# adolfogonzalez3/maddpg

Hardware: AMD Instinct MI355X
Metric: env-steps/sec (end-to-end at the reference update cadence), simple_spread N=3, batch 1024 (higher is better)
Workload: dtype fp32

## Files before the change

include/maddpg_hip.h:

```cpp
#ifndef MADDPG_HIP_H
#define MADDPG_HIP_H

#include <stddef.h>
#include <stdint.h>

#ifdef __cplusplus
extern "C" {
#endif

#define MDP_MAX_AGENTS 8
#define MDP_ACT_DIM 5
#define MDP_MAX_UNITS 256
#define MDP_ABI_VERSION 5

enum mdp_scenario {
    MDP_SCN_NONE = 0,
    MDP_SCN_SIMPLE = 1,
    MDP_SCN_SPREAD = 2,
    MDP_SCN_ADVERSARY = 3,
    MDP_SCN_TAG = 4,
    MDP_SCN_SPEAKER_LISTENER = 5
};

enum mdp_which {
// ... 162 lines not shown

int64_t mdp_td3_bytes(const mdp_config* cfg);
int mdp_td3_enable(mdp_handle* h, void* buf_dev, int64_t bytes, int32_t policy_delay);
int mdp_td3_info(mdp_handle* h, int32_t agent, double out4[4]);

int mdp_minimax_enable(mdp_handle* h, const float* eps_host);
int mdp_minimax_info(mdp_handle* h, float* eps_out_host);
int mdp_minimax_debug_adv(mdp_handle* h, float* critic_adv_dev, float* actor_adv_dev);

enum mdp_approx_set { MDP_APX_NET = 0, MDP_APX_TARGET = 1, MDP_APX_M = 2, MDP_APX_V = 3, MDP_APX_GRAD = 4 };
int64_t mdp_approx_bytes(const mdp_config* cfg);
int mdp_approx_enable(mdp_handle* h, void* buf_dev, int64_t bytes, float lambda);
int mdp_approx_set_params(mdp_handle* h, int32_t observer, int32_t agent, int32_t which, const float* src, int64_t n);
int mdp_approx_get_params(mdp_handle* h, int32_t observer, int32_t agent, int32_t which, float* dst, int64_t n);
int mdp_approx_get_beta_powers(mdp_handle* h, int32_t observer, int32_t agent, float out2[2]);
int mdp_approx_set_beta_powers(mdp_handle* h, int32_t observer, int32_t agent, const float in2[2]);
int mdp_approx_info(mdp_handle* h, int32_t observer, int32_t agent, double out4[4]);
int mdp_approx_logits(mdp_handle* h, int32_t observer, int32_t agent, int32_t target, const float* obs_dev,
                      float* logits_dev, int32_t rows);
int mdp_approx_grad(mdp_handle* h, int32_t observer, const int32_t* idx_dev);
int mdp_approx_step(mdp_handle* h, int32_t observer, const int32_t* idx_dev);

enum mdp_kernel_kind {
    MDP_K_INDEX = 0, MDP_K_GATHER = 1, MDP_K_CRITIC_GRAD = 2, MDP_K_ACTOR_GRAD = 3,
    MDP_K_APPLY = 4, MDP_K_ROLLOUT = 5, MDP_K_REDUCE = 6, MDP_K_REDUCE_APPLY = 7,
    MDP_K_ALLREDUCE = 8,
    MDP_K_PER_SYNC = 9, MDP_K_PER_SAMPLE = 10, MDP_K_PER_UPDATE = 11,
    MDP_K_EVAL = 12,
    MDP_K_COUNT = 13
};
int mdp_prof_enable(mdp_handle* h, int32_t kind, int32_t on);
int mdp_grad_variant(mdp_handle* h, int32_t agent);
int mdp_grad_twin(mdp_handle* h);
int mdp_prof_read(mdp_handle* h, int32_t kind, double* total_ms, int64_t* launches);

#ifdef __cplusplus
}
#endif
#endif
```

maddpg_amd/_lib.py:

```python
import ctypes
import os
import re

import torch

HERE = os.path.dirname(os.path.abspath(__file__))
LIB_PATH = os.environ.get("MDP_LIB") or os.path.join(HERE, "libmaddpg_hip.so")
HEADER = os.path.join(os.path.dirname(HERE), "include", "maddpg_hip.h")

MAX_AGENTS = 8
ACT_DISCRETE, ACT_BOX = 0, 1
ACT_DIM = 5
BENCH_W = 8
MAX_UNITS = 256
ABI_VERSION = 5

SCN = {"none": 0, "simple": 1, "simple_spread": 2, "simple_adversary": 3, "simple_tag": 4,
       "simple_speaker_listener": 5}
WHICH = {"actor": 0, "critic": 1, "tgt_actor": 2, "tgt_critic": 3, "m_actor": 4, "v_actor": 5,
         "m_critic": 6, "v_critic": 7, "g_actor": 8, "g_critic": 9,
         "critic2": 10, "tgt_critic2": 11, "m_critic2": 12, "v_critic2": 13, "g_critic2": 14}
APX_WHICH = {"net": 0, "tgt": 1, "m": 2, "v": 3, "grad": 4}
REGION = {"theta": 0, "target": 1, "adam_m": 2, "adam_v": 3, "grad": 4, "replay": 5, "index": 6,
          "stats": 7, "env": 8, "eplog": 9, "beta": 10, "slab": 11, "ctl": 12}
# ... 60 lines not shown
    "mdp_synchronize": (ctypes.c_int, [_P]),
    "mdp_region": (ctypes.c_int, [_P, _I32, ctypes.POINTER(_I64), ctypes.POINTER(_I64)]),
    "mdp_tensor": (ctypes.c_int, [_P, _I32, _I32, _I32, ctypes.POINTER(MdpTensorInfo)]),
    "mdp_row_layout": (ctypes.c_int, [_P, _I32, _I32P]),
    "mdp_set_act_dims": (ctypes.c_int, [_P, _I32P]),
    "mdp_get_act_dims": (ctypes.c_int, [_P, _I32P]),
    "mdp_set_act_spaces": (ctypes.c_int, [_P, _I32P, _I32P]),
    "mdp_get_act_spaces": (ctypes.c_int, [_P, _I32P, _I32P]),
    "mdp_set_params": (ctypes.c_int, [_P, _I32, _I32, _F32P, _I64]),
    "mdp_get_params": (ctypes.c_int, [_P, _I32, _I32, _F32P, _I64]),
    "mdp_get_beta_powers": (ctypes.c_int, [_P, _I32, _I32, _F32P]),
    "mdp_set_beta_powers": (ctypes.c_int, [_P, _I32, _I32, _F32P]),
    "mdp_buffer_len": (_I64, [_P]),
    "mdp_buffer_add_rows": (ctypes.c_int, [_P, _P, _I64]),
    "mdp_buffer_put_agent": (ctypes.c_int, [_P, _I32, _P, _P, _I64]),
    "mdp_buffer_set_len": (ctypes.c_int, [_P, _I64, _I64]),
    "mdp_buffer_set_ring": (ctypes.c_int, [_P, _I64, _I64, _I64]),
    "mdp_seed_py_random": (ctypes.c_int, [_P, ctypes.c_uint64]),
    "mdp_set_rng_state": (ctypes.c_int, [_P, _U32P]),
    "mdp_get_rng_state": (ctypes.c_int, [_P, _U32P]),
    "mdp_make_index": (ctypes.c_int, [_P, _I32, _P]),
    "mdp_sample_rows": (ctypes.c_int, [_P, _P, _I32, _P]),
    "mdp_act": (ctypes.c_int, [_P, _I32, _I32, _P, _P, _I32, _P]),
    "mdp_actor_logits": (ctypes.c_int, [_P, _I32, _I32, _P, _P, _I32]),
    "mdp_q_values": (ctypes.c_int, [_P, _I32, _I32, _P, _P, _I32]),
    "mdp_update": (ctypes.c_int, [_P, _I32, _P, _P, _P]),
    "mdp_update_gate": (ctypes.c_int, [_P, _I64]),
    "mdp_update_round": (ctypes.c_int, [_P]),
    "mdp_set_graphs": (ctypes.c_int, [_P, _I32]),
    "mdp_train_step": (ctypes.c_int, [_P, _I32]),
    "mdp_dp_unique_id": (ctypes.c_int, [ctypes.c_char_p]),
    "mdp_grad_variant": (ctypes.c_int, [_P, _I32]),
    "mdp_grad_twin": (ctypes.c_int, [_P]),
    "mdp_dp_init": (ctypes.c_int, [_P, ctypes.c_char_p, _I32, _I32]),
    "mdp_dp_xgmi_open": (ctypes.c_int, [_P, _I32, _I32, ctypes.c_char_p]),
    "mdp_dp_xgmi_connect": (ctypes.c_int, [_P, ctypes.c_char_p]),
    "mdp_dp_xgmi_probe": (ctypes.c_int, [_P, _I32P]),
    "mdp_dp_xgmi_enable": (ctypes.c_int, [_P]),
    "mdp_dp_xgmi_close": (ctypes.c_int, [_P]),
    "mdp_dp_info": (ctypes.c_int, [_P, _I32P]),
    "mdp_dp_exchange_stats": (ctypes.c_int, [_P, ctypes.POINTER(ctypes.c_double), _I32]),
    "mdp_dp_exchange_stats_enable": (ctypes.c_int, [_P, _I32]),
    "mdp_train_steps": (ctypes.c_int, [_P, _I32, ctypes.POINTER(ctypes.c_int32), _I32]),
    "mdp_agent_update": (ctypes.c_int, [_P, _I32, ctypes.c_int64, _P, _P, ctypes.POINTER(ctypes.c_double)]),
    "mdp_ra_plan": (ctypes.c_int, [ctypes.POINTER(MdpConfig), _I32, _I32, _I32P]),
    "mdp_critic_grad": (ctypes.c_int, [_P, _I32, _P, _P]),
    "mdp_actor_grad": (ctypes.c_int, [_P, _I32, _P, _P]),
    "mdp_reduce_grad": (ctypes.c_int, [_P, _I32, _I32]),
    "mdp_apply_grad": (ctypes.c_int, [_P, _I32, _I32, ctypes.c_float]),
    "mdp_get_stats": (ctypes.c_int, [_P, _I32, _F64P]),
    "mdp_check_finite": (ctypes.c_int, [_P, ctypes.POINTER(_I64)]),
    "mdp_env_reset": (ctypes.c_int, [_P]),
    "mdp_env_step": (ctypes.c_int, [_P, _P, _P]),
    "mdp_env_get_state": (ctypes.c_int, [_P, _F32P, _F32P, _I32P, _I32P]),
    "mdp_env_set_state": (ctypes.c_int, [_P, _F32P, _F32P, _I32P, _I32P]),
    "mdp_env_get_comm": (ctypes.c_int, [_P, _F32P]),
    "mdp_env_set_comm": (ctypes.c_int, [_P, _F32P]),
    "mdp_env_obs": (ctypes.c_int, [_P, _P]),
    "mdp_env_step_bench": (ctypes.c_int, [_P, _P]),
    "mdp_env_step_bench_u": (ctypes.c_int, [_P, _P, _P]),
    "mdp_evaluate": (ctypes.c_int, [_P, _I64, _I32, _I32, _P, _P, _P]),
    "mdp_evaluate_q": (ctypes.c_int, [_P, _I64, _I32, _I32, _I32, _I32, _P, _P, _P, _P, _P]),
    "mdp_eval_initial_state": (ctypes.c_int, [_P, _I64, _I32, _F32P, _F32P, _I32P]),
    "mdp_actor_set_floats": (_I64, [_P]),
    "mdp_actor_set_write": (ctypes.c_int, [_P, _P, _I32, _F32P, _I64]),
    "mdp_actor_set_snapshot": (ctypes.c_int, [_P, _P]),
# ... 79 lines not shown
```

maddpg_amd/csrc/mdp_api.cpp:

```cpp
#include <hip/hip_runtime.h>

#include <algorithm>
#include <cmath>
#include <cstdio>
#include <cstdlib>
#include <cstring>
#include <string>
#include <dlfcn.h>
#include <rccl/rccl.h>

#include <map>
#include <vector>

#include "mdp_kernels.h"
#include "mdp_variants.h"

namespace {

inline int64_t r4(int64_t n) { return (n + 3) & ~int64_t(3); }
inline int64_t a256(int64_t n) { return (n + 255) & ~int64_t(255); }

NDesc make_net(int64_t& off, int in, int H, int out) {
  NDesc d;
  d.off = (int)off;
// ... 251 lines not shown
}

struct mdp_handle {
  mdp_config cfg;
  Layout L;
  int device = 0;
  hipStream_t stream = nullptr;
  bool own_stream = false;
  char* arena = nullptr;
  float *theta, *target, *m, *v, *grad, *replay, *beta, *slab_c, *slab_a, *eplog;
  float *pos, *vel, *ep_rew;
  float* env_comm = nullptr;
  int32_t *index, *goal, *ep_step;
  double *stats, *stat_c, *stat_a, *y;
  Ctl* ctl;
  int64_t len = 0, next = 0;
  uint32_t act_ctr = 0, reset_ctr = 0;
  bool env_lockstep = true;
  std::string err;
  bool ready = false;
  bool prof_on[MDP_K_COUNT] = {};
  std::vector<hipEvent_t> ev[MDP_K_COUNT];
  size_t ev_used[MDP_K_COUNT] = {};
  double prof_ms[MDP_K_COUNT] = {};
  int64_t prof_n[MDP_K_COUNT] = {};
  bool graphs = true;
  bool capturing = false;
  int eager_rounds = 0;
  bool general_grads = false;
  bool box = false;
  bool fused_apply = true;
  bool ra_lanes = true;
  bool grad_twin = true;
  uint32_t* ra_ctr = nullptr;
  uint64_t* ra_part = nullptr;
  float* apre = nullptr;
  bool actor_pre = true;
  float* cpre = nullptr;
  bool critic_pre = true;
  float* apre_rows = nullptr;
  float* cpre_rows = nullptr;
  std::map<std::vector<int>, hipGraphExec_t> graph_exec;
  int eager_steps = 0;
  ncclComm_t comm = nullptr;
  int dp_world = 1;
  bool dp_graphs = false;
  int update_mode = 0;
  FusedApplyArgs* tp_list = nullptr;
  RaBatch tp_batch;
  RaBatch tp_reduce, tp_step;
  int ra_cap = 0, ra_batch_cap = 0;
  bool tp_fits[4] = {true, true, true, true};
  std::vector<FusedApplyArgs> tp_host[4];
  RaBatch tp_xchg;
  RaBatch tp_pair[3][MDP_MAX_AGENTS];
  bool tp_pair_fits[3][MDP_MAX_AGENTS] = {};
  FusedApplyArgs tp_pair_host[3][MDP_MAX_AGENTS][2];
  bool rollout_draw = true;
  bool draw_ahead = true;
  bool grad_pair = true;
  uint64_t* xbuf = nullptr;
  int x_world = 0, x_rank = 0;
  std::vector<void*> x_opened;
  XchgDesc* xd_dev = nullptr;
  uint32_t* x_probe = nullptr;
  uint32_t x_probe_ep = 0;
// ... 415 lines not shown
    if (lds > MDP_LDS_BUDGET) return fail(h, "minimax critic step does not fit in LDS");
    for (int j = 0; j < MDP_MAX_AGENTS; ++j) m.eps[j] = h->mm_eps[agent][j];
    m.adv_out = h->mm_adv_c;
    HIPCHK(h, mdp_launch_critic_grad_mm(m, h->L.topo.H, lds, h->stream));
    return 0;
  }
  if (lds_critic_bytes(h->L.topo, a.group) > MDP_LDS_BUDGET) return fail(h, "critic step does not fit in LDS");
  if (apx_agent(h, agent) && !tp) {
    CriticArgsApx x;
    static_cast<CriticArgs&>(x) = a;
    x.apx_target = apx_base(h, agent, MDP_APX_TARGET);
    HIPCHK(h, mdp_launch_critic_grad_apx(x, h->L.topo.H, lds_critic_bytes(h->L.topo, a.group), h->stream));
    return 0;
  }
  if (h->variant == Variant::Per && !tp)
    HIPCHK(h, mdp_launch_critic_grad_per(per_critic_args(h, a), h->L.topo.H, lds_critic_bytes(h->L.topo, a.group),
                                         h->stream));
  else
    HIPCHK(h, mdp_launch_critic_grad(a, h->L.topo.H, lds_critic_bytes(h->L.topo, a.group), h->stream));
  return 0;
}

ActorArgs actor_args(mdp_handle* h, int agent, const int32_t* idx, const float* u_act, bool tp, bool apre,
                     int pre_next, const int32_t* pre_idx, bool shared) {
  ActorArgs a;
  a.apre = apre ? h->apre : nullptr;
  a.apre_rows = h->apre_rows;
  a.cpre = nullptr;
  a.cpre_rows = h->cpre_rows;
  a.cpre_agent = pre_next;
  a.cpre_idx = pre_idx;
  a.target = h->target;
  a.multi = tp ? 2 : 0;
  a.slab_agent_stride = 0;
  a.topo = h->L.topo;
  a.agent = agent;
  a.B = h->cfg.batch_size;
  a.theta = h->theta;
  a.replay = h->replay;
  a.idx = idx;
  a.u_act = u_act;
  a.seed = h->cfg.seed;
  a.ctl = h->ctl;
  a.neg_inv_b = -1.0f / (float)a.B;
  a.reg_scale = (float)(2.0 * (double)h->cfg.actor_reg / ((double)a.B * MDP_ACT_DIM));
  a.slab = h->slab_a;
  a.slab_stride = h->L.slab_a;
  a.slab_stat = h->stat_a;
  if (tp) {
    if (!shared) a.slab += (int64_t)agent * h->L.nwg * h->L.slab_a;
    a.slab_stat += (int64_t)agent * h->L.nwg * 8;
  }
  return a;
}

int do_actor_grad(mdp_handle* h, int agent, const int32_t* idx, const float* u_act, bool tp = false,
                  bool apre = false, int pre_next = -1, const int32_t* pre_idx = nullptr, bool shared = false) {
  ActorArgs a = actor_args(h, agent, idx, u_act, tp, apre, pre_next, pre_idx, shared);
  ProfScope p(h, MDP_K_ACTOR_GRAD);
  if (!tp && !h->general_grads && grads_r_ok(h->L.topo, agent)) {
    int lds = lds_actor_r_bytes(h->L.topo);
    if (pre_next >= 0) {
      a.cpre = h->cpre;
      lds = std::max(lds, lds_critic_pre_bytes(h->L.topo));
    }
    HIPCHK(h, mdp_launch_actor_grad_r(a, lds, h->stream));
    return 0;
  }
  if (mm_agent(h, agent) && !tp) {
    ActorArgsMm m;
    static_cast<ActorArgs&>(m) = a;
    for (int j = 0; j < MDP_MAX_AGENTS; ++j) m.eps[j] = h->mm_eps[agent][j];
    m.adv_out = h->mm_adv_a;
    HIPCHK(h, mdp_launch_actor_grad_mm(m, h->L.topo.H, lds_actor_mm_bytes(h->L.topo), h->stream));
    return 0;
  }
  HIPCHK(h, mdp_launch_actor_grad(a, h->L.topo.H, lds_actor_bytes(h->L.topo), h->stream));
  return 0;
}

struct OptNet {
  NDesc net, other;
  float *theta, *target, *m, *v, *grad;
  const float* slab;
  int slab_stride;
  float* beta;
  const double* slab_stat;
  const double* y;
  double* stats_out;
  uint32_t* ticket;
  uint32_t* ctr;
  uint64_t* part;
  int slot;
  int net_id;
  int polyak, stats_mode, bump_ctr;
  bool own;
};

// ... 540 lines not shown
    a.slab_stat = h->stat_c;
    a.y_out = h->y;
    a.group = 0;
    a.twin = 1;
    a.multi = n;
    a.slab_agent_stride = nwg * h->L.slab_c;
    ProfScope p(h, MDP_K_CRITIC_GRAD);
    HIPCHK(h, mdp_launch_critic_grad_r(a, lds_c, h->stream));
  }
  {
    ActorArgs a;
    a.apre = nullptr;
    a.apre_rows = nullptr;
    a.cpre = nullptr;
    a.cpre_rows = nullptr;
    a.cpre_agent = -1;
    a.cpre_idx = nullptr;
    a.target = h->target;
    a.topo = h->L.topo;
    a.agent = 0;
    a.B = h->cfg.batch_size;
    a.theta = h->theta;
    a.replay = h->replay;
    a.idx = idx;
    a.u_act = u_act;
    a.seed = h->cfg.seed;
    a.ctl = h->ctl;
    a.neg_inv_b = -1.0f / (float)a.B;
    a.reg_scale = (float)(2.0 * (double)h->cfg.actor_reg / ((double)a.B * MDP_ACT_DIM));
    a.slab = h->slab_a;
    a.slab_stride = h->L.slab_a;
    a.slab_stat = h->stat_a;
    a.multi = n;
    a.slab_agent_stride = nwg * h->L.slab_a;
    ProfScope p(h, MDP_K_ACTOR_GRAD);
    HIPCHK(h, mdp_launch_actor_grad_r(a, lds_actor_r_bytes(h->L.topo), h->stream));
  }
  return 0;
}

int launch_tp_pair(mdp_handle* h, int pp, int i, int32_t* piece) {
  const int B = h->cfg.batch_size;
  const int kind = pp == 1 ? MDP_K_REDUCE : MDP_K_REDUCE_APPLY;
  if (h->tp_pair_fits[pp][i]) {
    RaBatch rb = h->tp_pair[pp][i];
    if (piece) {
      rb.pf_out = piece;
      rb.pf_count = B;
      rb.pf_ctl = h->ctl;
    }
    ProfScope p(h, kind);
    HIPCHK(h, mdp_launch_reduce_apply_batch(rb, h->stream));
    return 0;
  }
  for (int k = 0; k < 2; ++k) {
    FusedApplyArgs f = h->tp_pair_host[pp][i][k];
    if (piece) {
      f.pf_out = piece + (k ? (B + 1) / 2 : 0);
      f.pf_count = k ? B - (B + 1) / 2 : (B + 1) / 2;
      f.pf_ctl = h->ctl;
    }
    ProfScope p(h, kind);
    HIPCHK(h, mdp_launch_reduce_apply(f, h->stream, h->ra_lanes));
  }
  return 0;
}
// ... 321 lines not shown
  std::string err;
  if (!build_layout(cfg, L, err) || cus < 0 || per_cu < 0) return -1;
  int fallback = 0;
  for (int i = 0; i < cfg->n_agents; ++i)
    for (int net = 0; net < 2; ++net) {
      const int g = mdp_ra_grid_of(L.topo, i, net);
      const bool ok = mdp_ra_fits(L.topo, i, net, cus * per_cu);
      if (out) out[2 * i + net] = ok ? g : -g;
      fallback += ok ? 0 : 1;
    }
  return fallback;
}

int mdp_create(const mdp_config* cfg, void* arena_dev, int64_t arena_bytes, void* hip_stream, mdp_handle** out) {
  if (!out) return -1;
  *out = nullptr;
  mdp_handle* h = new mdp_handle();
  std::string err;
  if (!build_layout(cfg, h->L, err)) {
    h->err = err;
    *out = h;
    return -1;
  }
  h->cfg = *cfg;
  {
    const char* g = getenv("MDP_GENERAL_GRADS");
    h->general_grads = g && g[0] == '1';
    const char* u = getenv("MDP_UNFUSED_APPLY");
    h->fused_apply = !(u && u[0] == '1');
    const char* rl = getenv("MDP_RA_LANES");
    h->ra_lanes = !(rl && rl[0] == '0');
    const char* gt = getenv("MDP_GRAD_TWIN");
    h->grad_twin = !(gt && gt[0] == '0');
    const char* rd = getenv("MDP_ROLLOUT_DRAW");
    h->rollout_draw = !(rd && rd[0] == '0');
    const char* da = getenv("MDP_DRAW_AHEAD");
    h->draw_ahead = !(da && da[0] == '0');
    const char* gp = getenv("MDP_GRAD_PAIR");
    h->grad_pair = !(gp && gp[0] == '0');
    const char* ap = getenv("MDP_ACTOR_PRE");
    h->actor_pre = !(ap && ap[0] == '0');
    const char* cp = getenv("MDP_CRITIC_PRE");
    h->critic_pre = !(cp && cp[0] == '0');
  }
  if (!arena_dev || arena_bytes < h->L.total) {
    h->err = "arena missing or too small";
    *out = h;
    return -1;
  }
  *out = h;
  HIPCHK(h, hipGetDevice(&h->device));
  if (need_dev(h, arena_dev, h->L.total, "mdp_create", "arena_dev", false)) return -1;
  {
    int cus = 0, per = 0, per_b = 0;
    HIPCHK(h, hipDeviceGetAttribute(&cus, hipDeviceAttributeMultiprocessorCount, h->device));
    HIPCHK(h, mdp_ra_occupancy(&per));
    HIPCHK(h, mdp_ra_batch_occupancy(&per_b));
    h->ra_cap = cus * per;
    h->ra_batch_cap = cus * per_b;
    int scratch = 0;
    HIPCHK(h, mdp_spin_kernels_scratch(&scratch));
    if (scratch > 0) h->ra_cap = h->ra_batch_cap = 0;
    if (2 * h->L.nwg + h->L.nwg + 1 > cus) h->grad_twin = false;
  }
  if (hip_stream) {
    h->stream = (hipStream_t)hip_stream;
  } else {
    HIPCHK(h, hipStreamCreateWithFlags(&h->stream, hipStreamNonBlocking));
    h->own_stream = true;
  }
  h->arena = (char*)arena_dev;
  auto R = [&](int r) { return (void*)(h->arena + h->L.off[r]); };
  h->theta = (float*)R(MDP_R_THETA);
  h->target = (float*)R(MDP_R_TARGET);
  h->m = (float*)R(MDP_R_ADAM_M);
  h->v = (float*)R(MDP_R_ADAM_V);
  h->grad = (float*)R(MDP_R_GRAD);
  h->replay = (float*)R(MDP_R_REPLAY);
  h->index = (int32_t*)R(MDP_R_INDEX);
  h->stats = (double*)R(MDP_R_STATS);
  h->eplog = (float*)R(MDP_R_EPLOG);
  h->beta = (float*)R(MDP_R_BETA);
  h->ctl = (Ctl*)R(MDP_R_CTL);
  {
    const int E = cfg->num_envs, ne = h->L.n_ent, n = cfg->n_agents;
    char* p = (char*)R(MDP_R_ENV);
    h->pos = (float*)p;
    p += 4 * (int64_t)E * ne * 2;
    h->vel = (float*)p;
    p += 4 * (int64_t)E * ne * 2;
    h->goal = (int32_t*)p;
    p += 4 * (int64_t)E;
    h->ep_step = (int32_t*)p;
    p += 4 * (int64_t)E;
    h->ep_rew = (float*)p;
    p += 4 * (int64_t)E * n;
// ... 501 lines not shown
static bool any_prof(const mdp_handle* h) {
  for (int k = 0; k < MDP_K_COUNT; ++k)
    if (h->prof_on[k]) return true;
  return false;
}

int mdp_update_round(mdp_handle* h) {
  MDP_NEED(h);
  if (h->len <= 0) return fail(h, "update round on an empty replay buffer");
  h->trained = true;
  if (!h->graphs || any_prof(h) || h->eager_rounds < 1) {
    ++h->eager_rounds;
    td3_begin(h);
    const int rc = round_launches(h);
    if (!rc) commit_rounds(h, 1);
    return rc;
  }
  hipGraphExec_t x = nullptr;
  const int rc = captured_graph(h, graph_key(h, 0, {}), [&] { return round_launches(h); }, &x);
  if (rc) return rc;
  HIPCHK(h, hipGraphLaunch(x, h->stream));
  commit_rounds(h, 1);
  return 0;
}

int mdp_grad_variant(mdp_handle* h, int32_t agent) {
  if (unusable(h) || agent < 0 || agent >= h->cfg.n_agents) return -1;
  return (!h->general_grads && grads_r_ok(h->L.topo, agent)) ? 1 : 0;
}

int mdp_grad_twin(mdp_handle* h) {
  if (unusable(h)) return -1;
  return h->grad_twin ? 2 : 1;
}

int mdp_dp_unique_id(uint8_t* out128) {
  if (!out128 || !rccl().ok) return -1;
  ncclUniqueId id;
  if (rccl().get_id(&id) != ncclSuccess) return -1;
  std::memcpy(out128, &id, sizeof(id));
  return 0;
}

int mdp_dp_init(mdp_handle* h, const uint8_t* id128, int32_t world, int32_t rank) {
  if (unusable(h) || !id128) return -1;
  if (gate(h, Seam::DpInit)) return -1;
  if (h->p2p || h->xbuf) return fail(h, "mdp_dp_init: the xGMI exchange is already set up");
  if (!rccl().ok) return fail(h, "librccl.so.1 could not be loaded");
  if (world < 1 || rank < 0 || rank >= world) return fail(h, "mdp_dp_init: bad world/rank");
  if (h->comm) return fail(h, "mdp_dp_init: already initialised");
  ncclUniqueId id;
  std::memcpy(&id, id128, sizeof(id));
  HIPCHK(h, hipSetDevice(h->device));
  const ncclResult_t r = rccl().init_rank(&h->comm, world, id, rank);
  if (r != ncclSuccess) {
    h->comm = nullptr;
    h->err = std::string("ncclCommInitRank: ") + rccl().err(r);
    return -1;
  }
  h->dp_world = world;
  const char* g = getenv("MDP_DP_GRAPHS");
  h->dp_graphs = g && g[0] == '1';
  destroy_graphs(h, false);
  return 0;
}

// ... 1245 lines not shown
```

maddpg_amd/csrc/mdp_grads_r.hip:

```cpp
#include "mdp_device.h"
#include "mdp_kernels.h"
#include "mdp_mt.h"

#define MDP_RW MDP_R

#ifdef MDP_BUDGET
#ifndef MDP_BUDGET_AGENT
#define MDP_BUDGET_AGENT 1
#endif
#define MDP_BUD_N 72
#define MDP_BUD_WG 256
__device__ unsigned long long g_bud[2][MDP_BUD_WG][MDP_BUD_N];
__shared__ int s_bud;
__shared__ unsigned long long s_bud_t[MDP_BUD_N];
__shared__ unsigned s_bud_cnt;
#ifndef MDP_BUDGET_REP
#define MDP_BUDGET_REP 1
#endif
__device__ __forceinline__ unsigned long long bud_now() {
  const unsigned long long t = __builtin_amdgcn_s_memtime();
#if MDP_BUDGET_REP > 1
  const unsigned long long t2 = __builtin_amdgcn_s_memtime();
  asm volatile("" ::"s"(t2));
#endif
  return t;
}
__device__ __forceinline__ unsigned long long bud_real() { return __builtin_amdgcn_s_memrealtime(); }
#define BUD(i)                                           \
  do {                                                   \
    const unsigned long long t__ = bud_now();            \
    if ((threadIdx.x & 63) == 0) s_bud_t[i] = t__;       \
  } while (0)
// ... 801 lines not shown
    if (tt == 0 && half == 0) {
      s_l = sum16(s_l);
      s_y = sum16(s_y);
      s_r = sum16(s_r);
      s_q = sum16(s_q);
      if (lane == 0) {
        double* st = slab_stat + (int64_t)bx * 8;
        st[0] = s_l;
        st[1] = s_y;
        st[2] = s_r;
        st[3] = s_q;
      }
    }
  }
  const int vw = wave + 8 * half, vn = 8 * twin;
  CRIT_T(0);
  wgrad_vwaves(h1c, LH, RH, d2, LD, RH, slab + nd.t[2].off, vw, vn);
  CRIT_T(1);
  wgrad_vwaves(rowbuf + xo_c, ldr, ka_c, d1, LD, RH, slab + nd.t[0].off, vw, vn);
  CRIT_T(2);
  if (kb_c) wgrad_vwaves(rowbuf + ag.act_off, ldr, kb_c, d1, LD, RH, slab + nd.t[0].off + ka_c * RH, vw, vn);
  CRIT_T(3);
  if (wave == 4) MDP_STAMPW(9);
  if (vw == vn - 3) colsum64(d2, LD, slab + nd.t[3].off);
  if (vw == vn - 1) colsum64(d1, LD, slab + nd.t[1].off);
  CRIT_T(4);
  MDP_STAMP(10);
  MDP_WG_END(0);
}


template <bool NARROW>
__global__ __launch_bounds__(512) void k_actor_grad_r(ActorArgs a) {
  MDP_KARG_TOUCH("s"(a.agent), "s"(a.slab_stride), "s"(a.cpre_agent), "s"(a.topo.n), "s"(gridDim.x));
  if constexpr (NARROW) MDP_KARG_TOUCH("s"(a.topo.act_w4));
  extern __shared__ __attribute__((aligned(16))) float lds[];
  __shared__ int rows_ready;
  __shared__ int fwd_issued;
  BUD_BEGIN(1, a.agent, a.multi);
  MDP_WG_START(1);
  MDP_TL(a.ctl, 2, 0);
  int agent = a.agent, bx = blockIdx.x;
  if (a.cpre) {
    const int nwg = (a.B + MDP_RW - 1) / MDP_RW;
    if (bx >= nwg) {
      MDP_TL_ROLE(2, 1);
      critic_pre_tile<NARROW>(a, lds, &rows_ready, bx - nwg);
      MDP_WG_END(1);
      return;
    }
  }
  if (a.multi > 1) {
    const int nwg = (a.B + MDP_RW - 1) / MDP_RW;
    agent = bx / nwg;
    bx -= agent * nwg;
  }
  const int32_t* idx = a.multi > 1 ? a.idx + (int64_t)agent * a.B : a.idx;
  const float* u_act = (a.multi > 1 && a.u_act) ? a.u_act + (int64_t)agent * a.B * MDP_ACT_DIM : a.u_act;
  const Topo& T = a.topo;
  MDP_KARG_TOUCH(MDP_KARG_ADESC(T.ag[agent]));
  const ADesc& ag = T.ag[agent];
  const NDesc& na = ag.actor;
  const NDesc& nc = ag.critic;
  const bool lq = ag.local_q != 0;
  const int ldr = lds_ld(T.row_stride);
  const int ka_c = lq ? ag.obs_dim : ag.cin;
  const int xo_c = lq ? ag.obs_off : 0;
  LdsCarve cv(lds);
  MDP_CARVE_ACTOR_R(MDP_CARVE_DECL, ldr)

  const int wave = __builtin_amdgcn_readfirstlane(threadIdx.x >> 6);
  const int lane = threadIdx.x & 63, r = lane & 15, kq = lane >> 4;
  const int r0 = bx * MDP_R;
  const int nvalid = min(MDP_R, a.B - r0);
  const uint32_t ctr = ctr_load(a.ctl) + (a.multi > 1 ? (uint32_t)agent : 0u);
  const float* P = a.theta;
  constexpr int KC = 28, KSC = KC / 4;
  const int64_t ao = a.multi > 1 ? (int64_t)agent : 0;
  float* slab = a.slab + ao * a.slab_agent_stride + (int64_t)bx * a.slab_stride - na.off;
  double* slab_stat = a.slab_stat + ao * (int64_t)((a.B + MDP_R - 1) / MDP_R) * 8;
  MDP_STAMP(16);
  if (threadIdx.x == 0) rows_ready = 0;
  if (threadIdx.x == 1) fwd_issued = 0;
  __syncthreads();

  double s_q = 0.0, s_p = 0.0;
// ... 38 lines not shown
      if (lane < MDP_R) qv[lane] = ((qpart[lane] + qpart[MDP_R + lane]) + qpart[2 * MDP_R + lane]) +
                                   qpart[3 * MDP_R + lane] + P[nc.t[5].off];
      __syncthreads();
      MDP_STAMP(23);
      {
        const f32x4 acc = rdg_acc(d1c, LD, wda);
        if (r < MDP_ACT_DIM) {
#pragma unroll
          for (int i = 0; i < 4; ++i) da[(kq * 4 + i) * 8 + r] = acc[i];
        }
      }
      wave_sync();
      if (lane < MDP_R) {
        const int aw = act_w_of<NARROW>(T, agent);
        const float reg_scale = aw == MDP_ACT_DIM ? a.reg_scale : T.reg_scale_w[aw - 1];
        float dot = 0.f;
        for (int k = 0; k < MDP_ACT_DIM; ++k) dot += da[lane * 8 + k] * av[lane * 8 + k];
        for (int k = 0; k < MDP_ACT_DIM; ++k) {
          const float g = (da[lane * 8 + k] - dot) * av[lane * 8 + k] + lg[lane * 8 + k] * reg_scale;
          dl[lane * 8 + k] = lane < nvalid ? g : 0.f;
        }
        if (lane < nvalid) {
          s_q = (double)qv[lane];
          for (int k = 0; k < MDP_ACT_DIM; ++k) {
            const double p = (double)lg[lane * 8 + k];
            s_p += p * p;
          }
        }
      }
      __syncthreads();
      d2a_rows(h2a, dl, w3a, d2a, gwpart, 0);
      MDP_STAMP(24);
      __syncthreads();
      dw3a_store(gwpart, dl, slab + na.t[4].off, slab + na.t[5].off);
    } else {
      if (wave > 1) {
        if (a.apre) load_rows16_part(a.apre_rows + (int64_t)r0 * T.row_stride, T.row_stride, rowbuf, ldr, 128, 384);
        else gather_rows16_part(a.replay, T.row_stride, idx, r0, nvalid, rowbuf, ldr, 128, 384);
      }
      if (wave > 1) lds_signal(&rows_ready);
      const int k0 = KC * (wave - 1);
      f32x4 w1[KSC];
      rf_load<KSC>(w1, P + nc.t[0].off + k0 * RH, max(min(ka_c - k0, KC), 0));
      f32x4 w1b[2], b1;
      if (wave == 1) {
        rf_load<2>(w1b, P + nc.t[0].off + ag.a_in_off * RH, MDP_ACT_DIM);
        b1 = ld4(P + nc.t[1].off + 4 * r);
      }
      float w2t[16];
      rt_load<16>(w2t, P + nc.t[2].off, RH, 16 * wave + r, RH);
      const float b2t = P[nc.t[3].off + 16 * wave + r], w3t = P[nc.t[4].off + 16 * wave + r];
      lds_signal(&fwd_issued);
      lds_wait(&rows_ready, 6);
      if (wave == 1) MDP_STAMPW(56);
      f32x4 acc[4];
      rf_zero(acc);
      if (k0 < ka_c)
        rf_acc<KSC>(acc, rowbuf + xo_c + k0, ldr, min(ka_c - k0, KC), w1, ag.a_in_off - k0,
                    ag.a_in_off + MDP_ACT_DIM - k0);
      if (wave == 1) MDP_STAMPW(57);
      if (wave == 3) MDP_STAMPW(58);
      if (wave > 1) {
        float* pp = l1part + ((wave - 2) * 64 + lane) * 16;
#pragma unroll
        for (int t = 0; t < 4; ++t) *reinterpret_cast<f32x4*>(pp + 4 * t) = acc[t];
      }
      __syncthreads();
      if (wave == 1) {
        MDP_STAMPW(19);
#pragma unroll
        for (int t = 0; t < 4; ++t) {
          acc[t] += *reinterpret_cast<const f32x4*>(l1part + lane * 16 + 4 * t);
          acc[t] += *reinterpret_cast<const f32x4*>(l1part + (64 + lane) * 16 + 4 * t);
        }
        rf_acc<2>(acc, av, 8, MDP_ACT_DIM, w1b);
        rf_store<true>(acc, b1, h1c, LH);
      }
      __syncthreads();
      critic_l2_tile(h1c, w2t, b2t, w3t, wave, nvalid, a.neg_inv_b, d2c, qpart);
      if (wave == 1) MDP_STAMPW(20);
      float w3a[MDP_ACT_DIM];
#pragma unroll
      for (int k = 0; k < MDP_ACT_DIM; ++k) w3a[k] = P[na.t[4].off + lane * MDP_ACT_DIM + k];
      __syncthreads();
      __syncthreads();
      __syncthreads();
      d2a_rows(h2a, dl, w3a, d2a, gwpart, wave);
      __syncthreads();
    }
    wgrad_multi<4>(WgJob{h1a, d2a, slab + na.t[2].off, LH, RH, LD, RH}, WgJob{nullptr, nullptr, nullptr, 0, 0, 0, 64},
                   WgJob{nullptr, nullptr, nullptr, 0, 0, 0, 64}, 0, 4);
    if (wave == 3) colsum64(d2a, LD, slab + na.t[3].off);
    __syncthreads();
  } else {
    const int tt = wave - 4;
    if (a.apre) load_rows16_part(a.apre_rows + (int64_t)r0 * T.row_stride, T.row_stride, rowbuf, ldr, 128, 384);
    else gather_rows16_part(a.replay, T.row_stride, idx, r0, nvalid, rowbuf, ldr, 128, 384);
    lds_signal(&rows_ready);
    f32x4 wc[4], wa[4];
    lds_wait(&fwd_issued, 4);
    rdg_load(wc, P + nc.t[2].off, 16 * tt + r, true);
    rdg_load(wa, P + na.t[2].off, 16 * tt + r, true);
    __syncthreads();
    __syncthreads();
    __syncthreads();
    if (tt == 0) MDP_STAMPW(21);
    dgrad_tile(d2c, wc, h1c, d1c, tt);
    __syncthreads();
    if (tt == 0) MDP_STAMPW(22);
    __syncthreads();
    __syncthreads();
    if (tt == 0) MDP_STAMPW(25);
    dgrad_tile(d2a, wa, h1a, d1a, tt);
    __syncthreads();
    if (tt == 0) MDP_STAMPW(26);
  }
  wgrad_waves(rowbuf + ag.obs_off, ldr, ag.obs_dim, d1a, LD, RH, slab + na.t[0].off, 0, 8);
  if (wave == 7) colsum64(d1a, LD, slab + na.t[1].off);
  if (wave == 0) {
    s_q = sum16(s_q);
    s_p = sum16(s_p);
    if (lane == 0) {
      double* st = slab_stat + (int64_t)bx * 8;
      st[0] = s_q;
      st[1] = s_p;
    }
  }
  MDP_STAMP(27);
  MDP_WG_END(1);
}

namespace {
int row_tiles(int B) { return (B + MDP_RW - 1) / MDP_RW; }
template <auto K, typename A>
hipError_t launch_r(const A& a, int lds, hipStream_t s, int extra) {
  return mdp_launch_lds<K>(dim3(row_tiles(a.B) * (a.multi > 1 ? a.multi : 1) + extra), dim3(512), lds, s, a);
}
bool topo_narrow(const Topo& t) {
  for (int j = 0; j < t.n; ++j)
    if (topo_act_w(t, j) != MDP_ACT_DIM) return true;
  return false;
}
int critic_extra(const CriticArgs& a) {
  return (a.twin > 1 && a.multi <= 1 ? row_tiles(a.B) : 0) + (a.apre ? row_tiles(a.B) : 0) + (a.pf_count > 0 ? 1 : 0);
}
}

hipError_t mdp_launch_critic_grad_r(const CriticArgs& a, int lds_bytes, hipStream_t s) {
  const int extra = critic_extra(a);
  if (topo_narrow(a.topo)) return launch_r<k_critic_grad_r<false, true, CriticArgs>>(a, lds_bytes, s, extra);
  return launch_r<k_critic_grad_r<false, false, CriticArgs>>(a, lds_bytes, s, extra);
}
hipError_t mdp_launch_critic_grad_r_per(const CriticArgsPer& a, int lds_bytes, hipStream_t s) {
  const int extra = critic_extra(a);
  if (topo_narrow(a.topo)) return launch_r<k_critic_grad_r<true, true, CriticArgsPer>>(a, lds_bytes, s, extra);
  return launch_r<k_critic_grad_r<true, false, CriticArgsPer>>(a, lds_bytes, s, extra);
}
hipError_t mdp_launch_actor_grad_r(const ActorArgs& a, int lds_bytes, hipStream_t s) {
  const int extra = a.cpre ? row_tiles(a.B) : 0;
  if (topo_narrow(a.topo)) return launch_r<k_actor_grad_r<true>>(a, lds_bytes, s, extra);
  return launch_r<k_actor_grad_r<false>>(a, lds_bytes, s, extra);
}

#ifdef MDP_TIMELINE
extern "C" int mdp_debug_tl_r(unsigned long long* out, int reset) {
  const size_t n = sizeof(unsigned long long) * MDP_TL_SLOTS * MDP_TL_WG * 2;
  if (reset) {
    void* p = nullptr;
    if (hipGetSymbolAddress(&p, HIP_SYMBOL(g_mdp_tl)) != hipSuccess) return -1;
    return hipMemset(p, 0, n) == hipSuccess && hipDeviceSynchronize() == hipSuccess ? 0 : -1;
  }
  return hipMemcpyFromSymbol(out, HIP_SYMBOL(g_mdp_tl), n) == hipSuccess ? 0 : -1;
}
#endif

#ifdef MDP_BUDGET
extern "C" int mdp_debug_budget(unsigned long long* out, int reset) {
  const size_t n = sizeof(unsigned long long) * 2 * MDP_BUD_WG * MDP_BUD_N;
  if (reset) {
    void* p = nullptr;
    if (hipGetSymbolAddress(&p, HIP_SYMBOL(g_bud)) != hipSuccess) return -1;
    return hipMemset(p, 0, n) == hipSuccess && hipDeviceSynchronize() == hipSuccess ? 0 : -1;
  }
  return hipMemcpyFromSymbol(out, HIP_SYMBOL(g_bud), n) == hipSuccess ? 0 : -1;
}
#endif
#ifdef MDP_STAMPS
extern "C" int mdp_debug_stamps_r(unsigned long long* out, int n) {
  return hipMemcpyFromSymbol(out, HIP_SYMBOL(g_mdp_stamps), sizeof(unsigned long long) * n) == hipSuccess ? 0 : -1;
}
extern "C" int mdp_debug_crit_times(unsigned long long* t) {
  return hipMemcpyFromSymbol(t, HIP_SYMBOL(g_crit_t), sizeof(unsigned long long) * 64 * 8 * 6) == hipSuccess ? 0 : -1;
// ... 10 lines not shown
```

maddpg_amd/csrc/mdp_kernels.h:

```cpp
#pragma once
#include <hip/hip_runtime.h>
#include <hip/hip_ext.h>
#include <stdint.h>

#include <type_traits>

#include "mdp_carve.h"
#include "mdp_topo.h"

struct CriticArgs {
  int agent, B;
  const float* theta;
  const float* target;
  const float* replay;
  const int32_t* idx;
  const float* u_tgt;
  uint64_t seed;
  const Ctl* ctl;
  double gamma;
  float inv_b;
  float* slab;
  int slab_stride;
  double* slab_stat;
  double* y_out;
// ... 34 lines not shown
};

struct ApproxArgs {
  int B, m, nwg;
  int agents[MDP_MAX_AGENTS];
  const float* phi;
  const float* replay;
  const int32_t* idx;
  float inv_b, lambda;
  float* slab;
  int slab_stride;
  double* slab_stat;
  Topo topo;
};

#define MDP_CPRE_W 212

#define MDP_APRE_W 144

struct ActorArgsHead {
  int agent, B;
  const float* theta;
  const float* replay;
  const int32_t* idx;
  const float* u_act;
  uint64_t seed;
  const Ctl* ctl;
  float neg_inv_b;
  float reg_scale;
  float* slab;
  int slab_stride;
  double* slab_stat;
  int multi;
  int64_t slab_agent_stride;
  const float* apre;
  const float* apre_rows;
  float* cpre;
  float* cpre_rows;
  int cpre_agent;
  const int32_t* cpre_idx;
  const float* target;
};
struct ActorArgs : ActorArgsHead {
  Topo topo;
};
struct ActorArgsMm : ActorArgs {
  float eps[MDP_MAX_AGENTS];
  float* adv_out;
};

struct GradPairArgs {
  CriticArgs c;
  ActorArgsHead x;
};

struct ReduceArgs {
  const float* slab;
  int nwg, slab_stride;
  float* grad;
  int64_t off, size;
  float* beta;
  float b1, b2;
  Ctl* ctl;
  int bump_ctr;
};

// ... 425 lines not shown
```

Before: 1.156 million.

## Split actor gradient work across twin workgroups per row tile

Adds a twin mode to the row-tiled actor gradient kernel that launches a second set of workgroups per row tile. One half computes the layer-2 weight gradient over all 8 waves, and the other half does the data-gradient back to layer 1 plus the layer-1 weight gradient, following a small deal table. The aim is to shorten the serial critical path of each actor-gradient workgroup by spreading its work over more CUs. In exchange both halves redo the forward/backward prefix, more workgroups are launched, and the mode is turned off when there are too few CUs. It is on by default and can be disabled with MDP_ACTOR_TWIN=0.

```diff
diff --git a/include/maddpg_hip.h b/include/maddpg_hip.h
--- a/include/maddpg_hip.h
+++ b/include/maddpg_hip.h
@@ -218,6 +218,7 @@
 int mdp_prof_enable(mdp_handle* h, int32_t kind, int32_t on);
 int mdp_grad_variant(mdp_handle* h, int32_t agent);
 int mdp_grad_twin(mdp_handle* h);
+int mdp_actor_twin(mdp_handle* h);
 int mdp_prof_read(mdp_handle* h, int32_t kind, double* total_ms, int64_t* launches);
 
 #ifdef __cplusplus
diff --git a/maddpg_amd/_lib.py b/maddpg_amd/_lib.py
--- a/maddpg_amd/_lib.py
+++ b/maddpg_amd/_lib.py
@@ -116,6 +116,7 @@
     "mdp_dp_unique_id": (ctypes.c_int, [ctypes.c_char_p]),
     "mdp_grad_variant": (ctypes.c_int, [_P, _I32]),
     "mdp_grad_twin": (ctypes.c_int, [_P]),
+    "mdp_actor_twin": (ctypes.c_int, [_P]),
     "mdp_dp_init": (ctypes.c_int, [_P, ctypes.c_char_p, _I32, _I32]),
     "mdp_dp_xgmi_open": (ctypes.c_int, [_P, _I32, _I32, ctypes.c_char_p]),
     "mdp_dp_xgmi_connect": (ctypes.c_int, [_P, ctypes.c_char_p]),
diff --git a/maddpg_amd/csrc/mdp_actor_deal.h b/maddpg_amd/csrc/mdp_actor_deal.h
--- /dev/null
+++ b/maddpg_amd/csrc/mdp_actor_deal.h
@@ -0,0 +1,29 @@
+#pragma once
+
+#if defined(__HIPCC__) || defined(__CUDACC__)
+#define MDP_DEAL_FN __host__ __device__ constexpr
+#else
+#define MDP_DEAL_FN constexpr
+#endif
+
+struct ActorDeal {
+  int dw2_w0;
+  int dw2_wn;
+  int dw2_t;
+  int db2_wave;
+  int dgrad;
+  int dw1_wn;
+  int dw1_t;
+  int db1_wave;
+  int row_wave;
+};
+
+MDP_DEAL_FN ActorDeal actor_deal(int twin, int half) {
+  if (twin <= 1) return ActorDeal{0, 4, 4, 3, 1, 8, 1, 7, 0};
+  if (half == 0) return ActorDeal{0, 8, 2, 7, 0, 0, 0, -1, 0};
+  return ActorDeal{0, 0, 0, -1, 1, 8, 1, 7, -1};
+}
+
+MDP_DEAL_FN int actor_deal_dw2_wave(const ActorDeal& d, int t) { return d.dw2_wn > 0 ? d.dw2_w0 + t % d.dw2_wn : -1; }
+MDP_DEAL_FN int actor_deal_dw1_wave(const ActorDeal& d, int t) { return d.dw1_wn > 0 ? t % d.dw1_wn : -1; }
+MDP_DEAL_FN int actor_deal_tiles(int K) { return ((K + 15) >> 4) * 4; }
diff --git a/maddpg_amd/csrc/mdp_api.cpp b/maddpg_amd/csrc/mdp_api.cpp
--- a/maddpg_amd/csrc/mdp_api.cpp
+++ b/maddpg_amd/csrc/mdp_api.cpp
@@ -307,6 +307,7 @@
   bool fused_apply = true;
   bool ra_lanes = true;
   bool grad_twin = true;
+  bool actor_twin = true;
   uint32_t* ra_ctr = nullptr;
   uint64_t* ra_part = nullptr;
   float* apre = nullptr;
@@ -788,6 +789,7 @@
   a.cpre_idx = pre_idx;
   a.target = h->target;
   a.multi = tp ? 2 : 0;
+  a.twin = 1;
   a.slab_agent_stride = 0;
   a.topo = h->L.topo;
   a.agent = agent;
@@ -820,6 +822,7 @@
       a.cpre = h->cpre;
       lds = std::max(lds, lds_critic_pre_bytes(h->L.topo));
     }
+    if (h->actor_twin) a.twin = 2;
     HIPCHK(h, mdp_launch_actor_grad_r(a, lds, h->stream));
     return 0;
   }
@@ -1426,6 +1429,7 @@
     a.slab_stride = h->L.slab_a;
     a.slab_stat = h->stat_a;
     a.multi = n;
+    a.twin = 1;
     a.slab_agent_stride = nwg * h->L.slab_a;
     ProfScope p(h, MDP_K_ACTOR_GRAD);
     HIPCHK(h, mdp_launch_actor_grad_r(a, lds_actor_r_bytes(h->L.topo), h->stream));
@@ -1813,6 +1817,8 @@
     h->ra_lanes = !(rl && rl[0] == '0');
     const char* gt = getenv("MDP_GRAD_TWIN");
     h->grad_twin = !(gt && gt[0] == '0');
+    const char* at = getenv("MDP_ACTOR_TWIN");
+    h->actor_twin = !(at && at[0] == '0');
     const char* rd = getenv("MDP_ROLLOUT_DRAW");
     h->rollout_draw = !(rd && rd[0] == '0');
     const char* da = getenv("MDP_DRAW_AHEAD");
@@ -1843,6 +1849,7 @@
     HIPCHK(h, mdp_spin_kernels_scratch(&scratch));
     if (scratch > 0) h->ra_cap = h->ra_batch_cap = 0;
     if (2 * h->L.nwg + h->L.nwg + 1 > cus) h->grad_twin = false;
+    if (2 * h->L.nwg + h->L.nwg > cus) h->actor_twin = false;
   }
   if (hip_stream) {
     h->stream = (hipStream_t)hip_stream;
@@ -2410,6 +2417,11 @@
 int mdp_grad_twin(mdp_handle* h) {
   if (unusable(h)) return -1;
   return h->grad_twin ? 2 : 1;
+}
+
+int mdp_actor_twin(mdp_handle* h) {
+  if (unusable(h)) return -1;
+  return h->actor_twin ? 2 : 1;
 }
 
 int mdp_dp_unique_id(uint8_t* out128) {
diff --git a/maddpg_amd/csrc/mdp_grads_r.hip b/maddpg_amd/csrc/mdp_grads_r.hip
--- a/maddpg_amd/csrc/mdp_grads_r.hip
+++ b/maddpg_amd/csrc/mdp_grads_r.hip
@@ -1,3 +1,4 @@
+#include "mdp_actor_deal.h"
 #include "mdp_device.h"
 #include "mdp_kernels.h"
 #include "mdp_mt.h"
@@ -865,7 +866,8 @@
 
 template <bool NARROW>
 __global__ __launch_bounds__(512) void k_actor_grad_r(ActorArgs a) {
-  MDP_KARG_TOUCH("s"(a.agent), "s"(a.slab_stride), "s"(a.cpre_agent), "s"(a.topo.n), "s"(gridDim.x));
+  MDP_KARG_TOUCH("s"(a.agent), "s"(a.slab_stride), "s"(a.cpre_agent), "s"(a.topo.n), "s"(gridDim.x), "s"(a.B),
+                 "s"(a.multi), "s"(a.twin));
   if constexpr (NARROW) MDP_KARG_TOUCH("s"(a.topo.act_w4));
   extern __shared__ __attribute__((aligned(16))) float lds[];
   __shared__ int rows_ready;
@@ -874,17 +876,23 @@
   MDP_WG_START(1);
   MDP_TL(a.ctl, 2, 0);
   int agent = a.agent, bx = blockIdx.x;
+  const int twin = a.twin;
+  const int nwg = (a.B + MDP_RW - 1) / MDP_RW;
   if (a.cpre) {
-    const int nwg = (a.B + MDP_RW - 1) / MDP_RW;
-    if (bx >= nwg) {
+    if (bx >= twin * nwg) {
       MDP_TL_ROLE(2, 1);
-      critic_pre_tile<NARROW>(a, lds, &rows_ready, bx - nwg);
+      critic_pre_tile<NARROW>(a, lds, &rows_ready, bx - twin * nwg);
       MDP_WG_END(1);
       return;
     }
   }
+  int half = 0;
+  if (twin > 1) {
+    half = bx >= nwg ? 1 : 0;
+    bx -= half * nwg;
+  }
+  const ActorDeal deal = actor_deal(twin, half);
   if (a.multi > 1) {
-    const int nwg = (a.B + MDP_RW - 1) / MDP_RW;
     agent = bx / nwg;
     bx -= agent * nwg;
   }
@@ -989,7 +997,7 @@
       d2a_rows(h2a, dl, w3a, d2a, gwpart, 0);
       MDP_STAMP(24);
       __syncthreads();
-      dw3a_store(gwpart, dl, slab + na.t[4].off, slab + na.t[5].off);
+      if (deal.row_wave == 0) dw3a_store(gwpart, dl, slab + na.t[4].off, slab + na.t[5].off);
     } else {
       if (wave > 1) {
         if (a.apre) load_rows16_part(a.apre_rows + (int64_t)r0 * T.row_stride, T.row_stride, rowbuf, ldr, 128, 384);
@@ -1045,10 +1053,14 @@
       d2a_rows(h2a, dl, w3a, d2a, gwpart, wave);
       __syncthreads();
     }
-    wgrad_multi<4>(WgJob{h1a, d2a, slab + na.t[2].off, LH, RH, LD, RH}, WgJob{nullptr, nullptr, nullptr, 0, 0, 0, 64},
-                   WgJob{nullptr, nullptr, nullptr, 0, 0, 0, 64}, 0, 4);
-    if (wave == 3) colsum64(d2a, LD, slab + na.t[3].off);
-    __syncthreads();
+    if (deal.dw2_t == 4) {
+      static_assert(actor_deal(1, 0).dw2_w0 == 0 && actor_deal(1, 0).dw2_wn == 4 && actor_deal(1, 0).dw2_t == 4,
+                    "the call below");
+      wgrad_multi<4>(WgJob{h1a, d2a, slab + na.t[2].off, LH, RH, LD, RH}, WgJob{nullptr, nullptr, nullptr, 0, 0, 0, 64},
+                     WgJob{nullptr, nullptr, nullptr, 0, 0, 0, 64}, 0, 4);
+      if (wave == deal.db2_wave) colsum64(d2a, LD, slab + na.t[3].off);
+    }
+    if (deal.dgrad) __syncthreads();
   } else {
     const int tt = wave - 4;
     if (a.apre) load_rows16_part(a.apre_rows + (int64_t)r0 * T.row_stride, T.row_stride, rowbuf, ldr, 128, 384);
@@ -1057,7 +1069,7 @@
     f32x4 wc[4], wa[4];
     lds_wait(&fwd_issued, 4);
     rdg_load(wc, P + nc.t[2].off, 16 * tt + r, true);
-    rdg_load(wa, P + na.t[2].off, 16 * tt + r, true);
+    if (deal.dgrad) rdg_load(wa, P + na.t[2].off, 16 * tt + r, true);
     __syncthreads();
     __syncthreads();
     __syncthreads();
@@ -1068,13 +1080,26 @@
     __syncthreads();
     __syncthreads();
     if (tt == 0) MDP_STAMPW(25);
-    dgrad_tile(d2a, wa, h1a, d1a, tt);
-    __syncthreads();
-    if (tt == 0) MDP_STAMPW(26);
-  }
-  wgrad_waves(rowbuf + ag.obs_off, ldr, ag.obs_dim, d1a, LD, RH, slab + na.t[0].off, 0, 8);
-  if (wave == 7) colsum64(d1a, LD, slab + na.t[1].off);
-  if (wave == 0) {
+    if (deal.dgrad) {
+      dgrad_tile(d2a, wa, h1a, d1a, tt);
+      __syncthreads();
+      if (tt == 0) MDP_STAMPW(26);
+    }
+  }
+  if (deal.dw2_t == 2) {
+    static_assert(actor_deal(2, 0).dw2_w0 == 0 && actor_deal(2, 0).dw2_wn == 8 && actor_deal(2, 0).dw2_t == 2,
+                  "the call below");
+    wgrad_multi<2>(WgJob{h1a, d2a, slab + na.t[2].off, LH, RH, LD, RH}, WgJob{nullptr, nullptr, nullptr, 0, 0, 0, 64},
+                   WgJob{nullptr, nullptr, nullptr, 0, 0, 0, 64}, 0, 8);
+    if (wave == deal.db2_wave) colsum64(d2a, LD, slab + na.t[3].off);
+  }
+  if (deal.dw1_t == 1) {
+    static_assert(actor_deal(1, 0).dw1_wn == 8 && actor_deal(1, 0).dw1_t == 1, "the call below");
+    static_assert(actor_deal(2, 1).dw1_wn == 8 && actor_deal(2, 1).dw1_t == 1, "the call below");
+    wgrad_waves(rowbuf + ag.obs_off, ldr, ag.obs_dim, d1a, LD, RH, slab + na.t[0].off, 0, 8);
+    if (wave == deal.db1_wave) colsum64(d1a, LD, slab + na.t[1].off);
+  }
+  if (wave == deal.row_wave) {
     s_q = sum16(s_q);
     s_p = sum16(s_p);
     if (lane == 0) {
@@ -1114,7 +1139,7 @@
   return launch_r<k_critic_grad_r<true, false, CriticArgsPer>>(a, lds_bytes, s, extra);
 }
 hipError_t mdp_launch_actor_grad_r(const ActorArgs& a, int lds_bytes, hipStream_t s) {
-  const int extra = a.cpre ? row_tiles(a.B) : 0;
+  const int extra = (a.twin > 1 && a.multi <= 1 ? row_tiles(a.B) : 0) + (a.cpre ? row_tiles(a.B) : 0);
   if (topo_narrow(a.topo)) return launch_r<k_actor_grad_r<true>>(a, lds_bytes, s, extra);
   return launch_r<k_actor_grad_r<false>>(a, lds_bytes, s, extra);
 }
diff --git a/maddpg_amd/csrc/mdp_kernels.h b/maddpg_amd/csrc/mdp_kernels.h
--- a/maddpg_amd/csrc/mdp_kernels.h
+++ b/maddpg_amd/csrc/mdp_kernels.h
@@ -90,6 +90,7 @@
   int slab_stride;
   double* slab_stat;
   int multi;
+  int twin;
   int64_t slab_agent_stride;
   const float* apre;
   const float* apre_rows;
```

Result: no change. 1.163 million (median of 6 runs) (+0.7%).
